# MPEGGroup/mpeg-pcc-tmc13

Hardware: AMD Instinct MI355X
Metric: RAHT forward+inverse attribute-transform Mpoints/s (bit-exact vs CPU reference) (higher is better)
Workload: dtype int64 (Q15 fixed point), int32 I/O; 1 GPU; subnode=1 pred=1 ext=1 qp34: RAHT forward+inverse, 1x1000000 Morton-sorted S-lidar/GPU, C=1; frames_per_gpu=1, roundtrip_decoder_equals_encoder_recon=True

## Files before the change

mpeg-pcc-tmc13_amd/csrc/gpcc_attr_mi355.hip:

```cpp
#include <hip/hip_runtime.h>

#include <algorithm>
#include <cstdio>
#include <cstdlib>
#include <dlfcn.h>
#include <cstring>
#include <atomic>
#include <map>
#include <mutex>
#include <thread>
#include <string>
#include <cmath>
#include <vector>

#include "gpcc_attr_mi355.h"
#include "raht_common.hpp"
#include "raht_edges.hpp"
#include "raht_levels.hpp"
#include "raht_rdoq.hpp"
#include "raht_subnode.hpp"
#include "raht_pipe.hpp"
#include "raht_sweep.hpp"
#include "raht_tile.hpp"
#include "raht_tree.hpp"
// ... 442 lines not shown
  bool links = false;
};

void
carve(Arena& ar, Plan& pl)
{
  ar.reset();
  const int n = pl.n, s = pl.s, c = pl.c, nlev = pl.nlev;
  pl.pt_off = ar.take<int32_t>(s + 1);
  pl.cap.assign(nlev, 0);
  for (int li = 0; li < nlev; li++) {
    int64_t cap = n;
    const int up = nlev - 1 - li;
    if (up < 11) {
      int64_t full = (int64_t)s << (3 * up);
      cap = std::min<int64_t>(cap, full);
    }
    pl.cap[li] = cap;
    pl.tv.cap[li] = (int32_t)cap;
    pl.tv.key[li] = ar.take<int64_t>(cap + 1);
    pl.tv.fp[li] = ar.take<int32_t>(cap + 2);
    pl.tv.fc[li] = ar.take<int32_t>(cap + 2);
    pl.tv.soff[li] = ar.take<int32_t>(s + 1);
  }
  pl.tv.nlev = nlev;
  pl.tv.num_slices = s;
  pl.tv.n_total = n;
  pl.tv.num_tiles = (n + kTilePoints - 1) / kTilePoints;
  pl.tv.pt_off = pl.pt_off;
  pl.tile_cnt = ar.take<uint32_t>((size_t)pl.tv.num_tiles * nlev);
  pl.tile_attr = ar.take<int32_t>((size_t)pl.tv.num_tiles * c);
  pl.sched = ar.take<SliceSched>(s);
  pl.worklist = ar.take<int32_t>((size_t)n + 1);
  pl.work_count = ar.take<int32_t>(kMaxLevels * 9);
  pl.scan_state = ar.take<unsigned long long>(1024);
  pl.pocc = pl.sub ? ar.take<uint8_t>((size_t)n + 1) : nullptr;
  pl.mbox = pl.sub ? ar.take<uint32_t>((size_t)n * c * 4) : nullptr;
  pl.rdoq_state = (pl.sub && pl.lossy) ? ar.take<unsigned long long>((size_t)n + 1) : nullptr;
  pl.params = ar.take<gpcc_raht_params>(1);
  for (int i = 0; i < 2; i++) {
    pl.rec[i] = ar.take<int64_t>((size_t)n * c);
    pl.rec_us[i] = ar.take<int64_t>((size_t)n * c);
    pl.nneigh[i] = ar.take<int32_t>(n);
    pl.dqp[i] = pl.has_qp ? ar.take<int32_t>((size_t)n * 2) : nullptr;
  }
  pl.attr_prefix = nullptr;
  pl.dup_hf = nullptr;
  pl.haar_lf.assign(nlev, nullptr);
  pl.asc_qp.assign(nlev, nullptr);
  pl.haar_lf_tab = nullptr;
  pl.asc_qp_tab = nullptr;
  if (pl.encoder && !pl.haar)
    pl.attr_prefix = ar.take<int32_t>(((size_t)n + 1) * c);
  if (pl.encoder && pl.haar) {
    pl.dup_hf = ar.take<int32_t>((size_t)n * c);
    pl.haar_lf_tab = ar.take<int32_t*>(nlev);
    for (int li = 0; li < nlev; li++)
      pl.haar_lf[li] = ar.take<int32_t>((size_t)(pl.cap[li] + 1) * c);
  }
  if (pl.has_qp) {
    pl.asc_qp_tab = ar.take<int32_t*>(nlev);
    for (int li = 0; li < nlev; li++)
      pl.asc_qp[li] = ar.take<int32_t>((size_t)(pl.cap[li] + 1) * 2);
  }
  pl.desc = nullptr;
  pl.ptrans = nullptr;
  if (pl.lossy) {
    pl.desc = ar.take<uint32_t>(n);
    pl.ptrans = pl.sub ? nullptr : ar.take<int64_t>((size_t)n * c);
// ... 365 lines not shown
      for (int li = 1; li < nlev; li++) {
        ac.li = li;
        ascend_level_kernel<C><<<grid_for(pl.cap[li], 256), 256, 0, st>>>(ac);
      }
      if (pl.has_qp)
        qp_root_kernel<<<(s + 63) / 64, 64, 0, st>>>(ac, pl.sched);
    }
  }

  LevelCtx lc{};
  lc.tv = tv;
  lc.params = pl.params;
  lc.sched = pl.sched;
  lc.attr_prefix = pl.attr_prefix;
  lc.haar_lf = (encoder && pl.haar) ? pl.haar_lf_tab : nullptr;
  lc.asc_qp = pl.has_qp ? pl.asc_qp_tab : nullptr;
  for (int i = 0; i < 2; i++) {
    lc.rec[i] = pl.rec[i];
    lc.rec_us[i] = pl.rec_us[i];
    lc.nneigh[i] = pl.nneigh[i];
    lc.dqp[i] = pl.dqp[i];
  }
  lc.coeffs = d_coeffs;
  lc.desc = pl.desc;
  lc.ptrans = pl.ptrans;
  lc.lut = ctx->d_lut;
  lc.worklist = pl.worklist;
  lc.work_count = pl.work_count;
  lc.scan_state = pl.scan_state;
  lc.pocc = pl.pocc;
  lc.mbox = pl.mbox;
  lc.ticket = pl.work_count + kMaxLevels;
  lc.error = ctx->d_error;
  HIP_TRY(hipMemsetAsync(pl.work_count, 0, kMaxLevels * 9 * sizeof(int32_t), st));
  HIP_TRY(hipMemsetAsync(pl.scan_state, 0, 1024 * sizeof(unsigned long long), st));
  if (pl.mbox)
    HIP_TRY(hipMemsetAsync(pl.mbox, 0, (size_t)n * C * 4 * sizeof(uint32_t), st));
  if (pl.rdoq_state)
    HIP_TRY(hipMemsetAsync(pl.rdoq_state, 0, ((size_t)n + 1) * sizeof(unsigned long long), st));
  lc.rdoq_state = pl.rdoq_state;
  lc.slice_l = pl.slice_l;

  RdoqCtx rc{};
  if (pl.lossy) {
    rc.tv = tv;
    rc.sched = pl.sched;
    rc.tile_base = pl.rtile_base;
    rc.num_tiles = pl.num_rtiles;
    rc.desc = pl.desc;
    rc.coeffs = d_coeffs;
    rc.slice_l = pl.slice_l;
    rc.state = pl.rtile_state;
    rc.c = C;
    HIP_TRY(hipMemsetAsync(pl.rtile_state, 0, ((size_t)pl.num_rtiles + 1) * sizeof(unsigned long long), st));
    HIP_TRY(hipMemsetAsync(pl.slice_l, 0xff, 2 * (size_t)s * sizeof(int32_t), st));
  }

  if (tiles) {
    lc.li = 0;
    const int cgrid = std::min(s, 2048);
    if (!encoder) {
      Timer t(ctx, "coarse_synth");
      raht_coarse_kernel<C, kCoarseDecode><<<cgrid, 1024, 0, st>>>(lc);
    } else if (pl.haar) {
      Timer t(ctx, "coarse_fused");
      raht_coarse_kernel<C, kCoarseHaar><<<cgrid, 1024, 0, st>>>(lc);
    } else {
      Timer t(ctx, "coarse_lossy");
      raht_coarse_kernel<C, kCoarseLossy><<<cgrid, 1024, 0, st>>>(lc);
    }
  }

  HIP_TRY(hipEventSynchronize(ctx->ev_stats));
  const TreeStats ts = *ctx->h_stats;
  const int first_level = std::min(nlev - 1, tiles ? ts.fine_levels : ts.max_top);

  bool piped = false;
  if (pl.pipe && first_level >= 1) {
    PipeCtx px{};
    int64_t total = 0;
    for (int li = 0; li <= first_level; li++) {
      px.uoff[li] = (int32_t)total;
      total += ts.nodes[li];
    }
    const size_t need = (size_t)total * (4 + 1 + 4 + 32 * C) + 2048;
    void* pipe_mem = nullptr;
    if (total * C * 16 < ((int64_t)1 << 31) && pool_malloc(ctx, &pipe_mem, need) == hipSuccess) {
      Arena pa;
// ... 14 lines not shown
        Timer t(ctx, "pipe_prepass");
        pipe_iota_kernel<<<grid_for(total, 256), 256, 0, st>>>(px.src, (int)total);
        for (int li = first_level - 1; li >= 0; li--) {
          lc.li = li;
          const int64_t parents = ts.nodes[li + 1];
          raht_pipe_prepass_kernel<C><<<(int)std::min<int64_t>((parents + 1023) / 1024, 1024), 256, 0, st>>>(lc, px);
        }
      }
      {
        Timer t(ctx, "pipe_synth");
        if (pl.f64)
          raht_pipe_synth_kernel<C, ArithF64><<<kSubGrid, 256, 0, st>>>(lc, px);
        else
          raht_pipe_synth_kernel<C><<<kSubGrid, 256, 0, st>>>(lc, px);
      }
      {
        Timer t(ctx, "pipe_leaf");
        pipe_leaf_kernel<C><<<grid_for(ts.nodes[0], 256), 256, 0, st>>>(lc, px);
      }
      piped = true;
      pool_free(ctx, pipe_mem);
    }
  }

  LinkSchedule links;
  auto link_prof = [&](const char* name, int li) { return Timer(ctx, li < 0 ? name : level_name(name, li)); };
  const bool use_links = pl.links && !piped && !tiles && first_level >= 1 && hp->raht_extension != 0;
  if (use_links) {
    links.tv = tv;
    links.lv = pl.lv;
    links.begin(st, ts.nodes, first_level, link_prof);
  }
  int level_from = first_level;
  static const int rec_mode = [] {
    const char* e = getenv("GPCC_REC");
    return e ? atoi(e) : 0;
  }();
  const bool ext_flag = hp->raht_extension != 0;
  const bool use_rec = pl.sub && !pl.haar && !pl.has_qp && !pl.links && !piped && rec_mode == 1;
  size_t rec_need = 0;
  if (use_rec)
    for (int li = std::min(first_level, sweep ? std::max(0, ts.fine_levels) : first_level) - 1; li >= 0; li--)
      rec_need = std::max(rec_need, sweep_rec_bytes(level_max_blocks(ts.nodes, li, ext_flag), C));
  if (sweep && !piped && ts.fine_levels < first_level) {
    const int lo = std::max(0, ts.fine_levels);
    const SweepCtx sw{first_level - 1, lo};
    SweepRec rec{};
    const int64_t sweep_parents = sweep_rec_layout(&rec, ts.nodes, sw.li_hi, sw.li_lo);
    if (ensure_sweep_mem(ctx, std::max(rec_need, sweep_rec_bytes(sweep_parents, C))) == GPCC_OK) {
      level_from = lo;
      sweep_rec_carve(&rec, ctx->sweep_mem, sweep_parents, C);
      Timer t(ctx, encoder ? "sub_sweep_lossy" : "sub_sweep_synth");
      sweep_launch<C>(st, lc, sw, rec, ts.nodes, s, encoder, pl.f64);
    }
  }
  for (int li = piped ? -1 : level_from - 1; li >= 0; li--) {
    lc.li = li;
    lc.mtag = (uint32_t)(li + 1);
    const int64_t parents = ts.nodes[li + 1];
    if (use_links) {
      links.produce(st, li + 1, link_prof);
      lc.link_rec = pl.lv.rec[(li + 1) & 1];
      lc.link_lrec = pl.lv.lrec[(li + 1) & 1];
    }
    if (tiles) {
      const bool sparse = ts.nodes[li] * 8 <= parents * 9 && parents >= 64 * kTileTSparse;
      const int tile_t = sparse ? kTileTSparse : kTileT;
      const int ntiles = (int)((parents + tile_t - 1) / tile_t);
      const int tgrid = std::min((ntiles + 7) / 8 * 8, kLevelGridMax);
#define GPCC_TILE_LAUNCH(MODE)                                                  \
  do {                                                                          \
    if (sparse)                                                                 \
      raht_tile_kernel<C, MODE, kTileTSparse><<<tgrid, kTileThreads, 0, st>>>(lc); \
    else                                                                        \
      raht_tile_kernel<C, MODE, kTileT><<<tgrid, kTileThreads, 0, st>>>(lc);    \
  } while (0)
      if (!encoder) {
        Timer t(ctx, level_name("tile_synth", li));
        GPCC_TILE_LAUNCH(kSynth);
      } else if (pl.haar) {
        Timer t(ctx, level_name("tile_fused", li));
        GPCC_TILE_LAUNCH(kFused);
      } else {
        {
          Timer t(ctx, level_name("tile_analyze", li));
          GPCC_TILE_LAUNCH(kAnalyze);
        }
        rc.li = li;
        {
          Timer t(ctx, "rdoq_resolve");
          rdoq_resolve_launch(rc, st);
        }
        {
          Timer t(ctx, level_name("tile_synth_rec", li));
          GPCC_TILE_LAUNCH(kSynthRec);
        }
      }
#undef GPCC_TILE_LAUNCH
      continue;
    }
    {
      Timer t(ctx, level_name("level_prepass", li));
      raht_level_prepass_kernel<C><<<(int)std::min<int64_t>((parents + 1023) / 1024, 1024), 256, 0, st>>>(lc);
    }
    const int sgrid = (int)std::min<int64_t>(
      kSubGrid, std::max<int64_t>(8, (parents / (GPCC_SUB_BLOCKS_PER_WG) + 7) / 8 * 8));
    lc.claim_rounds = sub_claim_rounds(encoder, pl.haar, parents);
    bool rec_level = false;
    if (use_rec && ensure_sweep_mem(ctx, rec_need) == GPCC_OK) {
      Timer t(ctx, level_name("level_record", li));
      lc.brec = level_record_launch<C>(st, lc, li, ctx->sweep_mem, level_max_blocks(ts.nodes, li, ext_flag), encoder, pl.f64);
      rec_level = true;
    }
    if (rec_level && !encoder) {
      Timer t(ctx, level_name("level_sub_synth", li));
      if (pl.f64)
        raht_level_sub_kernel<C, kSynth, ArithF64, false, true><<<sgrid, 256, 0, st>>>(lc);
      else
        raht_level_sub_kernel<C, kSynth, ArithI64, false, true><<<sgrid, 256, 0, st>>>(lc);
    } else if (rec_level) {
      Timer t(ctx, level_name("level_sub_lossy", li));
      if (pl.f64)
        raht_level_sub_kernel<C, kLossySub, ArithF64, false, true><<<sgrid, 256, 0, st>>>(lc);
      else
        raht_level_sub_kernel<C, kLossySub, ArithI64, false, true><<<sgrid, 256, 0, st>>>(lc);
    } else if (!encoder) {
      Timer t(ctx, level_name("level_sub_synth", li));
      if (pl.f64)
        raht_level_sub_kernel<C, kSynth, ArithF64><<<sgrid, 256, 0, st>>>(lc);
      else
        raht_level_sub_kernel<C, kSynth><<<sgrid, 256, 0, st>>>(lc);
    } else if (pl.haar) {
      Timer t(ctx, level_name("level_sub_fused", li));
      raht_level_sub_kernel<C, kFused><<<sgrid, 256, 0, st>>>(lc);
// ... 3206 lines not shown
    while ((int64_t(3) << (shift << 1)) < dist2 && shift < 20)
      ++shift;
    *shift_bits = shift;
  } while (0);
  pool_free(ctx, d_xyz);
  pool_free(ctx, d_dist);
  return rc;
}

}

#if GPCC_FIN_VAR == 2
extern "C" int
gpcc_debug_fin(unsigned int* out, int reset)
{
  if (hipMemcpyFromSymbol(out, HIP_SYMBOL(gpcc::g_fin_dbg), sizeof(gpcc::g_fin_dbg)) != hipSuccess)
    return -1;
  if (reset) {
    unsigned int z[4 + 4 * 60] = {};
    if (hipMemcpyToSymbol(HIP_SYMBOL(gpcc::g_fin_dbg), z, sizeof(z)) != hipSuccess)
      return -1;
  }
  return 0;
}
#endif

#ifdef GPCC_SUB_PROF
extern "C" int
gpcc_debug_sub_prof(unsigned long long* out, int reset)
{
  if (hipMemcpyFromSymbol(out, HIP_SYMBOL(gpcc::g_sub_prof), sizeof(gpcc::g_sub_prof)) != hipSuccess)
    return -1;
  if (reset) {
    static unsigned long long z[16 + 32 * 20] = {};
    if (hipMemcpyToSymbol(HIP_SYMBOL(gpcc::g_sub_prof), z, sizeof(z)) != hipSuccess)
      return -1;
  }
  return 0;
}
#endif

#ifdef GPCC_PIPE_PROF
extern "C" int
gpcc_debug_pipe_prof(unsigned long long* out, int reset)
{
  if (hipMemcpyFromSymbol(out, HIP_SYMBOL(gpcc::g_pipe_prof), sizeof(gpcc::g_pipe_prof)) != hipSuccess)
    return -1;
  if (reset) {
    static unsigned long long z[32 * 8] = {};
    if (hipMemcpyToSymbol(HIP_SYMBOL(gpcc::g_pipe_prof), z, sizeof(z)) != hipSuccess)
      return -1;
  }
  return 0;
}
#endif

#ifdef GPCC_TILE_PROF
extern "C" int
gpcc_debug_tile_prof(unsigned long long* out, int reset)
{
  if (hipMemcpyFromSymbol(out, HIP_SYMBOL(gpcc::g_tile_prof), sizeof(gpcc::g_tile_prof)) != hipSuccess)
    return -1;
  if (reset) {
    static unsigned long long z[5 * 24 * 8] = {};
    if (hipMemcpyToSymbol(HIP_SYMBOL(gpcc::g_tile_prof), z, sizeof(z)) != hipSuccess)
      return -1;
  }
// ... 2676 lines not shown
```

mpeg-pcc-tmc13_amd/csrc/raht_levels.hpp:

```cpp
#pragma once

#include "raht_common.hpp"

namespace gpcc {

enum LevelMode { kAnalyze = 0, kSynth = 1, kFused = 2, kLossySub = 3 };

constexpr uint32_t kDescNever = 0x7fffffffu;
constexpr uint32_t kDescZero = 0x80000000u;

typedef const __attribute__((address_space(4))) gpcc_raht_params* ParamsConst;

struct InterRef {
  const int64_t* pos;
  const int32_t* prefix;
  int32_t n_ref;
  int32_t lr;
  int32_t blocks;
  int32_t dual;
  int32_t filtered;
  const int32_t* tap;
  const int64_t* hkey;
  const int32_t* hfp;
  const int32_t* hlf;
// ... 20 lines not shown


struct LevelCtx {
  TreeView tv;
  const gpcc_raht_params* params;
  const SliceSched* sched;
  const int32_t* attr_prefix;
  const int32_t* const* haar_lf;
  const int32_t* const* asc_qp;
  int64_t* rec[2];
  int64_t* rec_us[2];
  int32_t* nneigh[2];
  int32_t* dqp[2];
  int32_t* coeffs;
  uint32_t* desc;
  int64_t* ptrans;
  int32_t li;
  const struct SharedLut* lut;
  int32_t* worklist;
  int32_t* work_count;
  unsigned long long* scan_state;
  uint8_t* pocc;
  uint32_t* mbox;
  uint32_t mtag;
  int32_t* ticket;
  int32_t* error;
  unsigned long long* rdoq_state;
  int32_t* slice_l;
  InterRef inter;
  const int32_t* link_rec;
  const int32_t* link_lrec;
  int32_t claim_rounds;
  SweepRec brec;
};

template<typename T>
__device__ __forceinline__ T*
par2(T* const (&a)[2], int p)
{
  const ptrdiff_t d = a[1] - a[0];
  return a[0] + (p ? d : (ptrdiff_t)0);
}

constexpr int kSmallW = 16;
constexpr int kSmallN = 64;

struct SharedLut {
  RsqrtLut rsqrt;
  int32_t bfly_a[kSmallW * kSmallW];
  int32_t bfly_b[kSmallW * kSmallW];
  int32_t norm_rs[kSmallN];
  int32_t norm_sq[kSmallN];
};

__device__ __forceinline__ void
raht_coeffs_slow(int32_t wl, int32_t wr, const RsqrtLut& lut, int64_t* a, int64_t* b)
{
  const uint64_t rs = irsqrt((uint64_t)wl + (uint64_t)wr, lut);
  *a = (int64_t)(((uint64_t)isqrt((uint64_t)wl << 30, lut) * rs) >> 40);
  *b = (int64_t)(((uint64_t)isqrt((uint64_t)wr << 30, lut) * rs) >> 40);
}

__global__ __launch_bounds__(256) void
lut_init_kernel(SharedLut* g)
{
  __shared__ RsqrtLut rs;
// ... 265 lines not shown
          const int pt0 = tv.pt_off[s];
          const int64_t prow = (int64_t)pt0 + (j - tv.soff[li + 1][s]);
          const int64_t crow = (int64_t)pt0 + (c0 - tv.soff[li][s]);
          const int pp = e.parity ^ 1, cp = e.parity;
#pragma unroll
          for (int k = 0; k < C; k++) {
            par2(ctx.rec_us, cp)[crow * C + k] = par2(ctx.rec_us, pp)[prow * C + k];
            par2(ctx.rec, cp)[crow * C + k] = par2(ctx.rec, pp)[prow * C + k];
          }
          par2(ctx.nneigh, cp)[crow] = 19;
          if (ctx.asc_qp) {
            par2(ctx.dqp, cp)[crow * 2] = par2(ctx.dqp, pp)[prow * 2];
            par2(ctx.dqp, cp)[crow * 2 + 1] = par2(ctx.dqp, pp)[prow * 2 + 1];
          }
        } else {
          real = true;
        }
      }
    }
    const unsigned long long m = __ballot(real);
    __syncthreads();
    if (lane == 0)
      wave_cnt[wave] = __popcll(m);
    __syncthreads();
    int off = running;
    for (int w = 0; w < wave; w++)
      off += wave_cnt[w];
    if (real)
      ctx.worklist[off + __popcll(m & ((1ull << lane) - 1))] = j;
    running += wave_cnt[0] + wave_cnt[1] + wave_cnt[2] + wave_cnt[3];
  }
}

}
```

mpeg-pcc-tmc13_amd/csrc/raht_subnode.hpp:

```cpp
#pragma once

#include <stdlib.h>

#include "raht_arith.hpp"
#include "raht_inter.hpp"
#include "raht_levels.hpp"
#include "raht_links.hpp"

namespace gpcc {

#ifndef GPCC_SUB_CHUNK
#define GPCC_SUB_CHUNK 1
#endif
#ifndef GPCC_SUB_DSTORE
#define GPCC_SUB_DSTORE 0
#endif
__device__ __forceinline__ int64_t
sub_round_of_ticket(int tk, int cls)
{
  constexpr int K = GPCC_SUB_CHUNK;
  return ((int64_t)(tk / K) * 8 + cls) * K + tk % K;
}

#ifdef GPCC_SUB_PROF
__device__ unsigned long long g_sub_prof[16 + 32 * 20];
struct SubProf {
  unsigned long long t0 = 0, t1 = 0, last = 0, acc[4] = {0, 0, 0, 0}, iters = 0, idle_iters = 0;
  unsigned long long last2 = 0, sub_acc[6] = {0, 0, 0, 0, 0, 0}, execs[2] = {0, 0};
  template<int WHICH> __device__ void enter() { execs[WHICH]++; last2 = now(); }
  template<int K> __device__ void sub() { const unsigned long long t = now(); sub_acc[K] += t - last2; last2 = t; }
  __device__ static unsigned long long now() { return __builtin_amdgcn_s_memtime(); }
  __device__ void round_begin() { t0 = now(); }
  __device__ void loop_begin() { t1 = now(); }
  __device__ void iter_begin() { last = now(); iters++; }
  template<int STAGE> __device__ void mark() { const unsigned long long t = now(); acc[STAGE] += t - last; last = t; }
  __device__ void idle() { idle_iters++; }
  __device__ void round_end(int lane, int li)
  {
    if (lane != 0)
      return;
    const unsigned long long t2 = now();
    const unsigned long long v[9] = {1, t1 - t0, t2 - t1, acc[0], acc[1], acc[2], acc[3], iters, idle_iters};
    for (int i = 0; i < 9; i++)
      atomicAdd(&g_sub_prof[i], v[i]);
    atomicAdd(&g_sub_prof[16 + li * 4 + 0], 1ull);
    atomicAdd(&g_sub_prof[16 + li * 4 + 1], t1 - t0);
    atomicAdd(&g_sub_prof[16 + li * 4 + 2], t2 - t1);
    atomicAdd(&g_sub_prof[16 + li * 4 + 3], iters);
    for (int i = 0; i < 4; i++)
      atomicAdd(&g_sub_prof[144 + li * 6 + i], acc[i]);
    atomicAdd(&g_sub_prof[144 + li * 6 + 4], idle_iters);
    atomicAdd(&g_sub_prof[336 + li * 10 + 0], execs[0]);
    atomicAdd(&g_sub_prof[336 + li * 10 + 1], execs[1]);
    for (int i = 0; i < 6; i++)
      atomicAdd(&g_sub_prof[336 + li * 10 + 2 + i], sub_acc[i]);
  }
};
#else
struct SubProf {
  __device__ void round_begin() {}
  __device__ void loop_begin() {}
  __device__ void iter_begin() {}
  template<int STAGE> __device__ void mark() {}
  template<int WHICH> __device__ void enter() {}
  template<int K> __device__ void sub() {}
  __device__ void idle() {}
  __device__ void round_end(int, int) {}
};
#endif

inline int
sub_claim_rounds(bool encoder, bool haar, int64_t parents)
{
#if GPCC_EXPERIMENTS
  auto rounds = [] {
    const char* e = getenv("GPCC_SUB_CLAIM");
    const int v = e ? atoi(e) : 1;
    return v < 1 ? 1 : (v > 64 ? 64 : v);
  };
  auto limit = [] {
    const char* e = getenv("GPCC_SUB_CLAIM_PARENTS");
    return e ? (int64_t)atoll(e) : (int64_t)100000;
  };
#ifdef GPCC_EMU
  const int r = rounds();
  const int64_t lim = limit();
#else
  static const int r = rounds();
  static const int64_t lim = limit();
#endif
  return (encoder && !haar && r > 1 && parents <= lim) ? r : 1;
#else
  (void)encoder;
  (void)haar;
  (void)parents;
  return 1;
#endif
}

__device__ __forceinline__ int
occu_shift(int i12)
{
  constexpr uint8_t s[12] = {6, 5, 4, 3, 2, 1, 3, 1, 2, 1, 2, 3};
  return s[i12];
}

__device__ __forceinline__ int32_t
load_agent_i32(const int32_t* p)
{
  return __hip_atomic_load(p, __ATOMIC_RELAXED, __HIP_MEMORY_SCOPE_AGENT);
}
__device__ __forceinline__ int64_t
load_agent_i64(const int64_t* p)
{
  return __hip_atomic_load(p, __ATOMIC_RELAXED, __HIP_MEMORY_SCOPE_AGENT);
}
__device__ __forceinline__ void
store_agent_i64(int64_t* p, int64_t v)
{
  __hip_atomic_store(p, v, __ATOMIC_RELAXED, __HIP_MEMORY_SCOPE_AGENT);
}

#ifndef GPCC_SUB_SLEEP
#define GPCC_SUB_SLEEP 4
#endif
#ifndef GPCC_SUB_LOSSY_WAVES
#define GPCC_SUB_LOSSY_WAVES 3
#endif
#ifndef GPCC_SUB_SYNTH3_WAVES
#define GPCC_SUB_SYNTH3_WAVES 4
#endif
// ... 18 lines not shown
  const TreeView& tv = ctx.tv;
  const ParamsConst prm = (ParamsConst)ctx.params;
  const int li = ctx.li;
  const int t = threadIdx.x & 7;
  const int lane = lane_id();
  const int gbase = threadIdx.x & 56;
  const bool haar = !A::kF64 && prm->integer_haar_enable_flag != 0;
  const bool ext = A::kF64 || prm->raht_extension != 0;
  const int32_t epoch = li + 1;
#ifdef GPCC_EMU
  __shared__ unsigned long long wmail_s[8 * 4 * 64 * C];
  unsigned long long* wm = wmail_s + ((blockIdx.x & 7) * 4 + (threadIdx.x >> 6)) * (64 * C);
#else
  __shared__ unsigned long long wmail_s[4 * 64 * C];
  unsigned long long* wm = wmail_s + (threadIdx.x >> 6) * (64 * C);
#endif
#ifdef GPCC_EMU
  __shared__ int32_t nrow_s[8][12][256];
  __shared__ int32_t pwc_s[8 * 4][12];
#define GPCC_SUB_NROW(i12) nrow_s[blockIdx.x & 7][i12][threadIdx.x]
#define GPCC_SUB_PWC(i12) pwc_s[(blockIdx.x & 7) * 4 + (threadIdx.x >> 6)][i12]
#else
  __shared__ int32_t nrow_s[12][256];
  __shared__ int32_t pwc_s[4][12];
#define GPCC_SUB_NROW(i12) nrow_s[i12][threadIdx.x]
#define GPCC_SUB_PWC(i12) pwc_s[threadIdx.x >> 6][i12]
#endif
  if (lane < 12)
    GPCC_SUB_PWC(lane) = prm->pred_weight_child[lane];
  bool in_range = true;
  const int cls = blockIdx.x & 7;

  const int num_work = ctx.work_count[li];
#if GPCC_EXPERIMENTS
  const int claim_rounds = ctx.claim_rounds > 1 ? ctx.claim_rounds : 1;
  bool stop_all = false;
  for (;;) {
    int tk = 0;
    if (lane == 0)
      tk = atomicAdd(&ctx.ticket[li * 8 + (claim_rounds > 1 ? 0 : cls)], 1);
    tk = __shfl(tk, 0);
    const int64_t wround0 = claim_rounds > 1 ? (int64_t)tk * claim_rounds : sub_round_of_ticket(tk, cls);
    if (wround0 * 8 >= num_work || stop_all)
      break;
    bool carry_known = false;
    int carry_l = -1;
   for (int sr = 0; sr < claim_rounds; sr++) {
    const int64_t wround = wround0 + sr;
    if (wround * 8 >= num_work)
      break;
    SubProf prof;
    prof.round_begin();
    if (__hip_atomic_load(ctx.error, __ATOMIC_RELAXED, __HIP_MEMORY_SCOPE_AGENT)) {
      stop_all = true;
      break;
    }
#else
  for (;;) {
    int tk = 0;
    if (lane == 0)
      tk = atomicAdd(&ctx.ticket[li * 8 + cls], 1);
    tk = __shfl(tk, 0);
    const int64_t wround = sub_round_of_ticket(tk, cls);
    if (wround * 8 >= num_work)
      break;
    SubProf prof;
// ... 434 lines not shown
      }
    }

    int nb_c0[3] = {0, 0, 0};
    uint32_t nb_occ[3] = {0, 0, 0};
    int nb_single[3] = {0, 0, 0};
    VT nb_v[3][C];
#pragma unroll
    for (int slot = 0; slot < 3; slot++) {
#pragma unroll
      for (int k = 0; k < C; k++)
        nb_v[slot][k] = A::zero();
      const int i = 1 + t + 8 * slot;
      if (run && i >= 7 && i < 19 && pn[slot] >= 0) {
        const int q = pn[slot];
#pragma unroll
        for (int k = 0; k < C; k++) {
          nb_v[slot][k] = A::from_i64(prec[(rbase + q) * C + k]);
          in_range = in_range && A::below(nb_v[slot][k], A::kRecLimit);
        }
        if constexpr (REC) {
          nb_c0[slot] = rf[(kSfNbc0 + slot) * rln];
          nb_occ[slot] = (rpk >> (8 * slot)) & 0xffu;
          nb_single[slot] = (int)((rpk >> (24 + slot)) & 1u);
        } else if (q < j) {
          const int qc0 = tv.fc[li + 1][q];
          nb_c0[slot] = qc0;
          nb_occ[slot] = ctx.pocc[q];
          nb_single[slot] = ext && tv.fc[li + 1][q + 1] - qc0 == 1;
        }
      }
    }
    uint32_t pend = 0;
    uint32_t inw = 0, wsrc_a = 0, wsrc_b = 0;
    int jg[8];
#pragma unroll
    for (int g = 0; g < 8; g++)
      jg[g] = __shfl(on ? j : -1, g << 3);
#pragma unroll
    for (int i12 = 0; i12 < 12; i12++) {
      const int i = 7 + i12;
      const int owner = gbase | ((i - 1) & 7);
      const int sl = (i - 1) >> 3;
      const int q = __shfl(pn[sl], owner);
      const int qc0 = __shfl(nb_c0[sl], owner);
      const uint32_t qocc = __shfl(nb_occ[sl], owner);
      const int single = __shfl(nb_single[sl], owner);
      VT v[C];
#pragma unroll
      for (int k = 0; k < C; k++)
        v[k] = shfl_v(nb_v[sl][k], owner);
      if (!run || q < 0)
        continue;
      if (A::muli(v[0], 10) <= lim_lo || A::muli(v[0], 10) >= lim_hi)
        continue;
      if (has && ((neigh_mask(i) >> t) & 1)) {
        const int sh = occu_shift(i12);
        const int cpos = i12 < 9 ? t + sh : t - sh;
        const bool child_ok = cpos >= 0 && cpos < 8 && ((qocc >> cpos) & 1);
        if (child_ok) {
          const int cidx_n = qc0 + popc32(qocc & ((1u << cpos) - 1));
          const int64_t nrow = (int64_t)pt0 + (cidx_n - sc0);
          const int pwc = prm->pred_weight_child[i12];
          wsum += pwc;
          if (single) {
            const int mul = ext ? pwc : (pwc << kFpFrac);
#pragma unroll
            for (int k = 0; k < C; k++) {
              const VT cv = A::from_i64(par2(ctx.rec, cur_par)[nrow * C + k]);
              in_range = in_range && A::below(cv, A::kRecLimit);
              pred[k] += A::muli(cv, mul);
            }
          } else {
            GPCC_SUB_NROW(i12) = (int32_t)nrow;
            pend |= 1u << i12;
            int pg = -1;
#pragma unroll
            for (int g = 0; g < 7; g++)
              pg = q == jg[g] ? g : pg;
            if (pg >= 0) {
              inw |= 1u << i12;
              if (i12 < 10)
                wsrc_a |= (uint32_t)pg << (3 * i12);
              else
                wsrc_b |= (uint32_t)pg << (3 * (i12 - 10));
            }
          }
        } else {
          const int pwp = prm->pred_weight_parent[i];
          wsum += pwp;
          const int mul = ext ? pwp : (pwp << kFpFrac);
#pragma unroll
          for (int k = 0; k < C; k++)
            pred[k] += A::muli(v[k], mul);
        }
      }
    }
    const VC pdiv = A::coef(pred_divisor(wsum > 0 ? wsum : 1));
    const auto mrsrc = __builtin_amdgcn_make_buffer_rsrc(
      ctx.mbox, 0, (int)((size_t)tv.n_total * C * 16), 0x00020000);

    bool use_inter = false;
    VT ipin[C];
#pragma unroll
    for (int k = 0; k < C; k++)
      ipin[k] = A::zero();
    if constexpr (INTER) {
      if (ctx.inter.blocks) {
        bool node;
        int64_t pin[C];
        if (ctx.inter.hkey)
          inter_block_haar<C>(ctx.inter, on ? tv.key[li + 1][j] : 0, t, on, &node, pin);
        else
          inter_block<C>(ctx.inter, on ? tv.key[li + 1][j] : 0, t, on, lut, &node, pin);
        use_inter = node;
#pragma unroll
        for (int k = 0; k < C; k++) {
          ipin[k] = A::from_i64(pin[k]);
          in_range = in_range && (!node || A::below(ipin[k], A::kFwdLimit));
        }
        if (use_inter) {
          pend = 0;
          inw = 0;
          enable_pred = on;
        }
      }
    }

    int stage = on ? 0 : 3;
    unsigned spins = 0;
    VT pt[C];
    int32_t qc[C];
    uint32_t dr = kDescZero;
    int zs = 0;
    bool zero_r = false;
    uint32_t dmask = 0;
    bool lin_exact = false;
    int need = 0;
    int look = wi - 1;
    int outk = 0, outv = -1;
    unsigned long long done = 0;
    unsigned long long done_seen = ~0ull;
    int cur_slot = -1, cur_pwc = 0;
    int32_t cur_row = 0;
#pragma unroll
    for (int k = 0; k < C; k++) {
      pt[k] = A::zero();
      qc[k] = (!kEnc && coded) ? cplane[(size_t)k * n_s] : 0;
    }
#ifndef GPCC_EMU
    __builtin_amdgcn_s_waitcnt(0x0f70);
#endif
    prof.loop_begin();
    while (__any(stage != 3)) {
      bool progressed = false;
      prof.iter_begin();
      if (done != done_seen) {
        done_seen = done;
        uint32_t mi = stage == 0 ? (pend & inw) : 0u;
        while (__any(mi != 0)) {
          const bool act = mi != 0;
          const int slot = act ? __ffs(mi) - 1 : 0;
          mi &= mi - 1;
          const uint32_t pg = (slot < 10 ? wsrc_a >> (3 * slot) : wsrc_b >> (3 * (slot - 10))) & 7u;
          constexpr unsigned long long kShifts = 06ull | 05ull << 3 | 04ull << 6 | 03ull << 9 | 02ull << 12
            | 01ull << 15 | 03ull << 18 | 01ull << 21 | 02ull << 24 | 01ull << 27 | 02ull << 30 | 03ull << 33;
          const int sh = (int)((kShifts >> (3 * slot)) & 7);
          const int srcl = (int)(pg << 3) | ((slot < 9 ? t + sh : t - sh) & 7);
          if (act && ((done >> srcl) & 1)) {
            const int pwc = GPCC_SUB_PWC(slot);
            const int mul = ext ? pwc : (pwc << kFpFrac);
#pragma unroll
            for (int k = 0; k < C; k++)
              pred[k] += A::muli(__builtin_bit_cast(VT, wm[srcl * C + k]), mul);
            pend &= ~(1u << slot);
            inw &= ~(1u << slot);
          }
        }
      }
      const uint32_t pm = stage == 0 ? (pend & ~inw) : 0u;
      u32x4 g[C];
      if (pm) {
        const int slot = __ffs(pm) - 1;
        if (slot != cur_slot) {
          cur_slot = slot;
          cur_row = GPCC_SUB_NROW(slot);
          cur_pwc = GPCC_SUB_PWC(slot);
        }
#pragma unroll
        for (int k = 0; k < C; k++)
          g[k] = __builtin_amdgcn_raw_buffer_load_b128(mrsrc, (cur_row * C + k) * 16, 0,  16);
      }
      auto take_poll = [&]() -> bool {
        bool ok = pm != 0;
        if (pm) {
#pragma unroll
          for (int k = 0; k < C; k++) {
#ifndef GPCC_EMU
            asm volatile("" : : "v"(g[k]));
#endif
            ok = ok && g[k].z == ctx.mtag;
          }
          if (ok) {
            const int mul = ext ? cur_pwc : (cur_pwc << kFpFrac);
#pragma unroll
            for (int k = 0; k < C; k++)
              pred[k] += A::muli(__builtin_bit_cast(VT, ((uint64_t)g[k].y << 32) | g[k].x), mul);
            pend &= ~(1u << cur_slot);
          }
        }
        return ok;
      };
      bool blocked = group8_any(stage == 0 && pend);
      bool poll_open = __any(stage == 0 && !blocked);
      if (!poll_open) {
        if (__any(take_poll()))
          blocked = group8_any(stage == 0 && pend);
      }
      auto take_poll_behind = [&]() {
#ifndef GPCC_EMU
        __builtin_amdgcn_s_waitcnt(0x0f70);
#endif
        if (poll_open)
          take_poll();
      };
      prof.mark<0>();
      const bool nready = stage == 0 && !blocked;

      if (__any(nready)) {
        progressed = true;
        prof.template enter<0>();
        VT pw_[C];
#pragma unroll
        for (int k = 0; k < C; k++)
          pw_[k] = pred[k];
        if (run && has) {
#pragma unroll
          for (int k = 0; k < C; k++) {
            pw_[k] = A::mulc(pw_[k], pdiv);
            if constexpr (!A::kF64) {
              if (haar)
                pw_[k] = (pw_[k] >> kFpFrac) << kFpFrac;
            }
          }
        }
        if (!haar && w > 1 && enable_pred) {
#pragma unroll
          for (int k = 0; k < C; k++)
            pw_[k] = A::mulc(pw_[k], nrm_sq);
        }
#pragma unroll
        for (int k = 0; k < C; k++)
          in_range = in_range && A::below(pw_[k], A::kFwdLimit);
#pragma unroll
        for (int st = 0; st < 3; st++) {
          const int bit = 1 << st;
          const bool left = !(t & bit);
          const bool both = wl[st] && wr[st];
          const bool swap = !wl[st] && wr[st];
#pragma unroll
          for (int k = 0; k < C; k++) {
            const VT own = pw_[k], oth = shfl_xor_v(own, bit);
            if constexpr (A::kF64) {
              const VT bf = A::mulc(own, ca[st]) + A::mulc(left ? oth : -oth, cb[st]);
// ... 313 lines not shown
      if (!kLossy)
        take_poll_behind();
      if (__any(can)) {
        if (can && has) {
          VT vn[C];
#pragma unroll
          for (int k = 0; k < C; k++) {
            VT v = pw_[k];
            if (!haar && w > 1)
              v = A::mulc(A::shr(v, nrm_shift), nrm_rs);
            v = ext ? v : A::round_int(v);
            vn[k] = v;
            const uint64_t vb = __builtin_bit_cast(uint64_t, v);
            wm[lane * C + k] = vb;
            const u32x4 gr = {(uint32_t)vb, (uint32_t)(vb >> 32), ctx.mtag, 0u};
#if GPCC_SUB_DSTORE
            __builtin_amdgcn_raw_buffer_store_b128(gr, mrsrc, (int)((crow * C + k) * 16), 0, 0);
#endif
            __builtin_amdgcn_raw_buffer_store_b128(gr, mrsrc, (int)((crow * C + k) * 16), 0,  16);
          }
          prof.template sub<3>();
#pragma unroll
          for (int k = 0; k < C; k++) {
            par2(ctx.rec_us, cur_par)[crow * C + k] = A::to_i64(ext ? pw_[k] : A::round_int(A::muli(pw_[k], 4)));
            par2(ctx.rec, cur_par)[crow * C + k] = A::to_i64(vn[k]);
          }
          par2(ctx.nneigh, cur_par)[crow] = inherit_dc ? neigh_count : 19;
          prof.template sub<4>();
        }
        if (can)
          stage = 3;
      }

      done |= __ballot(can && has);
      prof.mark<3>();
      if (!progressed) {
        prof.idle();
        if (++spins > (1u << 21)) {
          if (lane == 0)
            atomicExch(ctx.error, 1);
          break;
        }
        __builtin_amdgcn_s_sleep(GPCC_SUB_SLEEP);
      }
    }
    prof.round_end(lane, li);
#if GPCC_EXPERIMENTS
    if (kLossy && claim_rounds > 1) {
      const unsigned long long fin = __ballot(outk == 2) & 0x0101010101010101ull;
      if (fin) {
        carry_l = __shfl(outv, 63 - __clzll((long long)fin));
        carry_known = true;
      } else if (__any(outk == 1)) {
        carry_known = false;
      }
    }
   }
#endif
  }
  if (A::kF64 && __any(!in_range) && lane == 0)
    atomicCAS(ctx.error, 0, 3);
#undef GPCC_SUB_NROW
#undef GPCC_SUB_PWC
}

}
```

Baseline: 101.3 Mpoints/s.

## Plan all RAHT levels in one kernel and copy single-child nodes in tail

Adds a single up-front planning kernel that builds per-level worklists and child-occupancy bytes for every level, using a decoupled look-back scan. This replaces the per-level prepass launches. Single-child parents are left out of the worklist, and the subnode kernel copies them with a ticketed, ILP-unrolled tail copy, also propagating slice_l for lossy mode. The single-neighbour prediction now reuses already-shuffled neighbour values instead of reloading rec, which drops the in-range check on that path. The planning kernel needs larger scan and pocc buffers and relies on cross-block spinning.

After: 97.28 Mpoints/s. 0.96x the previous value.

```diff
diff --git a/mpeg-pcc-tmc13_amd/csrc/gpcc_attr_mi355.hip b/mpeg-pcc-tmc13_amd/csrc/gpcc_attr_mi355.hip
--- a/mpeg-pcc-tmc13_amd/csrc/gpcc_attr_mi355.hip
+++ b/mpeg-pcc-tmc13_amd/csrc/gpcc_attr_mi355.hip
@@ -498,9 +498,9 @@
   pl.tile_attr = ar.take<int32_t>((size_t)pl.tv.num_tiles * c);
   pl.sched = ar.take<SliceSched>(s);
   pl.worklist = ar.take<int32_t>((size_t)n + 1);
-  pl.work_count = ar.take<int32_t>(kMaxLevels * 9);
-  pl.scan_state = ar.take<unsigned long long>(1024);
-  pl.pocc = pl.sub ? ar.take<uint8_t>((size_t)n + 1) : nullptr;
+  pl.work_count = ar.take<int32_t>(kMaxLevels * 17);
+  pl.scan_state = ar.take<unsigned long long>((size_t)kMaxLevels * kPlanScanRow);
+  pl.pocc = pl.sub ? ar.take<uint8_t>(std::max<size_t>((size_t)n + 1, (size_t)plan_pocc_offset(pl.tv.cap, nlev - 1) + 1)) : nullptr;
   pl.mbox = pl.sub ? ar.take<uint32_t>((size_t)n * c * 4) : nullptr;
   pl.rdoq_state = (pl.sub && pl.lossy) ? ar.take<unsigned long long>((size_t)n + 1) : nullptr;
   pl.params = ar.take<gpcc_raht_params>(1);
@@ -932,8 +932,16 @@
   lc.mbox = pl.mbox;
   lc.ticket = pl.work_count + kMaxLevels;
   lc.error = ctx->d_error;
-  HIP_TRY(hipMemsetAsync(pl.work_count, 0, kMaxLevels * 9 * sizeof(int32_t), st));
-  HIP_TRY(hipMemsetAsync(pl.scan_state, 0, 1024 * sizeof(unsigned long long), st));
+  static const int rec_mode = [] {
+    const char* e = getenv("GPCC_REC");
+    return e ? atoi(e) : 0;
+  }();
+  const bool ext_flag = hp->raht_extension != 0;
+  const bool planned = pl.sub && ext_flag && !pl.pipe && !pl.links && rec_mode != 1
+    && sub_claim_rounds(encoder, pl.haar, 0) == 1;
+  HIP_TRY(hipMemsetAsync(pl.work_count, 0, kMaxLevels * 17 * sizeof(int32_t), st));
+  HIP_TRY(hipMemsetAsync(
+    pl.scan_state, 0, (planned ? (size_t)nlev * kPlanScanRow : (size_t)kPlanScanRow) * sizeof(unsigned long long), st));
   if (pl.mbox)
     HIP_TRY(hipMemsetAsync(pl.mbox, 0, (size_t)n * C * 4 * sizeof(uint32_t), st));
   if (pl.rdoq_state)
@@ -954,6 +962,11 @@
     rc.c = C;
     HIP_TRY(hipMemsetAsync(pl.rtile_state, 0, ((size_t)pl.num_rtiles + 1) * sizeof(unsigned long long), st));
     HIP_TRY(hipMemsetAsync(pl.slice_l, 0xff, 2 * (size_t)s * sizeof(int32_t), st));
+  }
+
+  if (planned) {
+    Timer t(ctx, "level_plan");
+    raht_plan_levels_kernel<C><<<(int)std::min<int64_t>(((int64_t)n + 1023) / 1024, 1024), 256, 0, st>>>(lc);
   }
 
   if (tiles) {
@@ -1034,11 +1047,6 @@
     links.begin(st, ts.nodes, first_level, link_prof);
   }
   int level_from = first_level;
-  static const int rec_mode = [] {
-    const char* e = getenv("GPCC_REC");
-    return e ? atoi(e) : 0;
-  }();
-  const bool ext_flag = hp->raht_extension != 0;
   const bool use_rec = pl.sub && !pl.haar && !pl.has_qp && !pl.links && !piped && rec_mode == 1;
   size_t rec_need = 0;
   if (use_rec)
@@ -1101,7 +1109,11 @@
 #undef GPCC_TILE_LAUNCH
       continue;
     }
-    {
+    if (planned) {
+      lc.worklist = pl.worklist + plan_worklist_offset(ts.nodes[li + 1], ts.nodes[nlev - 1]);
+      lc.pocc = pl.pocc + plan_pocc_offset(pl.tv.cap, li);
+      lc.tail = 1;
+    } else {
       Timer t(ctx, level_name("level_prepass", li));
       raht_level_prepass_kernel<C><<<(int)std::min<int64_t>((parents + 1023) / 1024, 1024), 256, 0, st>>>(lc);
     }
diff --git a/mpeg-pcc-tmc13_amd/csrc/raht_levels.hpp b/mpeg-pcc-tmc13_amd/csrc/raht_levels.hpp
--- a/mpeg-pcc-tmc13_amd/csrc/raht_levels.hpp
+++ b/mpeg-pcc-tmc13_amd/csrc/raht_levels.hpp
@@ -76,6 +76,7 @@
   const int32_t* link_lrec;
   int32_t claim_rounds;
   SweepRec brec;
+  int32_t tail;
 };
 
 template<typename T>
@@ -407,4 +408,228 @@
   }
 }
 
-}
+__host__ __device__ inline int64_t
+plan_worklist_offset(int64_t nodes_parents, int64_t nodes_top)
+{
+  return nodes_parents - nodes_top;
+}
+__host__ __device__ inline int64_t
+plan_pocc_offset(const int32_t* cap, int li)
+{
+  int64_t o = 0;
+  for (int l = 0; l < li; l++)
+    o += (int64_t)cap[l + 1] + 1;
+  return o;
+}
+constexpr int kPlanScanRow = 1024;
+
+constexpr int kTailIlp = 4;
+constexpr int kTailChunk = kTailIlp * kWave;
+
+template<int C>
+__device__ __forceinline__ void
+level_copy_single_children(const LevelCtx& ctx, int li, int64_t j0, int lane, int num_parents)
+{
+  const TreeView& tv = ctx.tv;
+  bool one[kTailIlp];
+  int64_t prow[kTailIlp], crow[kTailIlp];
+  int cp[kTailIlp];
+#pragma unroll
+  for (int u = 0; u < kTailIlp; u++) {
+    const int64_t jj = j0 + lane + u * kWave;
+    const bool ok = jj < num_parents;
+    const int j = ok ? (int)jj : 0;
+    const int s = find_slice(tv.soff[li + 1], tv.num_slices, j);
+    const LevelSched e = ctx.sched[s].lvl[li];
+    const int c0 = tv.fc[li + 1][j];
+    const int c1 = tv.fc[li + 1][j + 1];
+    const int pt0 = tv.pt_off[s];
+    one[u] = ok && e.processed && c1 - c0 == 1;
+    prow[u] = (int64_t)pt0 + (j - tv.soff[li + 1][s]);
+    crow[u] = (int64_t)pt0 + (c0 - tv.soff[li][s]);
+    cp[u] = e.parity;
+  }
+  int64_t us[kTailIlp][C], sc[kTailIlp][C];
+  int32_t q0[kTailIlp], q1[kTailIlp];
+#pragma unroll
+  for (int u = 0; u < kTailIlp; u++) {
+    q0[u] = q1[u] = 0;
+#pragma unroll
+    for (int k = 0; k < C; k++)
+      us[u][k] = sc[u][k] = 0;
+    if (one[u]) {
+#pragma unroll
+      for (int k = 0; k < C; k++) {
+        us[u][k] = par2(ctx.rec_us, cp[u] ^ 1)[prow[u] * C + k];
+        sc[u][k] = par2(ctx.rec, cp[u] ^ 1)[prow[u] * C + k];
+      }
+      if (ctx.asc_qp) {
+        q0[u] = par2(ctx.dqp, cp[u] ^ 1)[prow[u] * 2];
+        q1[u] = par2(ctx.dqp, cp[u] ^ 1)[prow[u] * 2 + 1];
+      }
+    }
+  }
+#pragma unroll
+  for (int u = 0; u < kTailIlp; u++) {
+    if (one[u]) {
+#pragma unroll
+      for (int k = 0; k < C; k++) {
+        par2(ctx.rec_us, cp[u])[crow[u] * C + k] = us[u][k];
+        par2(ctx.rec, cp[u])[crow[u] * C + k] = sc[u][k];
+      }
+      par2(ctx.nneigh, cp[u])[crow[u]] = 19;
+      if (ctx.asc_qp) {
+        par2(ctx.dqp, cp[u])[crow[u] * 2] = q0[u];
+        par2(ctx.dqp, cp[u])[crow[u] * 2 + 1] = q1[u];
+      }
+    }
+  }
+}
+
+constexpr int kPlanIlp = 4;
+
+template<int C>
+__global__ __launch_bounds__(256) void
+raht_plan_levels_kernel(LevelCtx ctx)
+{
+  GPCC_VGPR_FLOOR_64();
+  __shared__ int wave_cnt[kPlanIlp][4];
+  __shared__ int base_s;
+  if (tree_failed(ctx.tv))
+    return;
+  const TreeView& tv = ctx.tv;
+  const bool ext = ctx.params->raht_extension != 0;
+  const int lane = lane_id(), wave = threadIdx.x >> 6;
+  const int64_t nodes_top = tv.soff[tv.nlev - 1][tv.num_slices];
+  for (int li = tv.nlev - 2; li >= 0; li--) {
+    const int num_parents = tv.soff[li + 1][tv.num_slices];
+    const int64_t seg = (int64_t)tv.soff[li][tv.num_slices] - num_parents;
+    int32_t* __restrict__ worklist = ctx.worklist + plan_worklist_offset(num_parents, nodes_top);
+    uint8_t* __restrict__ pocc = ctx.pocc + plan_pocc_offset(tv.cap, li);
+    unsigned long long* scan = ctx.scan_state + (size_t)li * kPlanScanRow;
+    const int32_t* __restrict__ fc = tv.fc[li + 1];
+    const int64_t* __restrict__ key = tv.key[li];
+    const int64_t chunks = ((int64_t)num_parents + 255) >> 8;
+    const int64_t per = (chunks + gridDim.x - 1) / gridDim.x;
+    const int active = per ? (int)((chunks + per - 1) / per) : 0;
+    if ((int)blockIdx.x >= active)
+      continue;
+    const int64_t gbeg = (int64_t)blockIdx.x * per;
+    const int64_t gend = min(gbeg + per, chunks);
+
+    int mine = 0;
+    for (int64_t chunk = gbeg; chunk < gend; chunk += kPlanIlp) {
+#pragma unroll
+      for (int u = 0; u < kPlanIlp; u++) {
+        const int64_t jj = (chunk + u) * 256 + threadIdx.x;
+        const bool ok = chunk + u < gend && jj < num_parents;
+        const int j = ok ? (int)jj : 0;
+        const int s = find_slice(tv.soff[li + 1], tv.num_slices, j);
+        const bool proc = ctx.sched[s].lvl[li].processed != 0;
+        const int nchild = fc[j + 1] - fc[j];
+        mine += ok && proc && !(ext && nchild == 1);
+      }
+    }
+#pragma unroll
+    for (int d = 1; d < kWave; d <<= 1)
+      mine += __shfl_xor(mine, d);
+    __syncthreads();
+    if (lane == 0)
+      wave_cnt[0][wave] = mine;
+    __syncthreads();
+    if (wave == 0) {
+      const unsigned long long ep = (unsigned long long)(li + 1) << 48;
+      const unsigned total = wave_cnt[0][0] + wave_cnt[0][1] + wave_cnt[0][2] + wave_cnt[0][3];
+      unsigned excl = 0;
+      if (blockIdx.x > 0) {
+        if (lane == 0)
+          __hip_atomic_store(&scan[blockIdx.x], ep | (1ull << 32) | total, __ATOMIC_RELAXED, __HIP_MEMORY_SCOPE_AGENT);
+        int base = (int)blockIdx.x - 1;
+        while (base >= 0) {
+          const int k = base - lane;
+          unsigned long long v = 0;
+          if (k >= 0)
+            v = __hip_atomic_load(&scan[k], __ATOMIC_RELAXED, __HIP_MEMORY_SCOPE_AGENT);
+          const bool valid = k >= 0 && (v >> 48) == (unsigned long long)(li + 1);
+          const unsigned long long inv = __ballot(k >= 0 && !valid);
+          const unsigned long long fin = __ballot(valid && ((v >> 32) & 0xffff) == 2);
+          const int first_inv = inv ? __ffsll((long long)inv) - 1 : kWave;
+          const int first_fin = fin ? __ffsll((long long)fin) - 1 : kWave;
+          if (first_inv < first_fin) {
+            __builtin_amdgcn_s_sleep(2);
+            continue;
+          }
+          unsigned part = (valid && lane <= first_fin) ? (unsigned)v : 0u;
+#pragma unroll
+          for (int d = 1; d < kWave; d <<= 1)
+            part += __shfl_xor(part, d);
+          excl += part;
+          if (first_fin < kWave)
+            break;
+          base -= kWave;
+        }
+      }
+      if (lane == 0) {
+        __hip_atomic_store(&scan[blockIdx.x], ep | (2ull << 32) | (excl + total), __ATOMIC_RELAXED, __HIP_MEMORY_SCOPE_AGENT);
+        if ((int)blockIdx.x == active - 1) {
+          ctx.work_count[li] = (int64_t)(excl + total) <= seg ? (int)(excl + total) : 0;
+          if ((int64_t)(excl + total) > seg)
+            atomicExch(ctx.error, 1);
+        }
+        base_s = (int)excl;
+      }
+    }
+    __syncthreads();
+    int running = base_s;
+
+    for (int64_t chunk = gbeg; chunk < gend; chunk += kPlanIlp) {
+      int j[kPlanIlp], c0[kPlanIlp], nchild[kPlanIlp];
+      bool proc[kPlanIlp];
+#pragma unroll
+      for (int u = 0; u < kPlanIlp; u++) {
+        const int64_t jj = (chunk + u) * 256 + threadIdx.x;
+        const bool ok = chunk + u < gend && jj < num_parents;
+        j[u] = ok ? (int)jj : 0;
+        const int s = find_slice(tv.soff[li + 1], tv.num_slices, j[u]);
+        proc[u] = ok && ctx.sched[s].lvl[li].processed != 0;
+        const int a = fc[j[u]], b = fc[j[u] + 1];
+        c0[u] = proc[u] ? a : 0;
+        nchild[u] = proc[u] ? b - a : 0;
+      }
+      unsigned long long m[kPlanIlp];
+      bool real[kPlanIlp];
+#pragma unroll
+      for (int u = 0; u < kPlanIlp; u++) {
+        uint32_t o = 0;
+#pragma unroll
+        for (int t = 0; t < 8; t++) {
+          const int64_t k8 = key[c0[u] + (t < nchild[u] ? t : 0)];
+          o |= t < nchild[u] ? 1u << (int)(k8 & 7) : 0u;
+        }
+        if (proc[u])
+          pocc[j[u]] = (uint8_t)o;
+        real[u] = proc[u] && !(ext && nchild[u] == 1);
+        m[u] = __ballot(real[u]);
+      }
+      __syncthreads();
+      if (lane == 0) {
+#pragma unroll
+        for (int u = 0; u < kPlanIlp; u++)
+          wave_cnt[u][wave] = __popcll(m[u]);
+      }
+      __syncthreads();
+#pragma unroll
+      for (int u = 0; u < kPlanIlp; u++) {
+        int off = running;
+        for (int w = 0; w < wave; w++)
+          off += wave_cnt[u][w];
+        const int at = off + __popcll(m[u] & ((1ull << lane) - 1));
+        if (real[u] && at < seg)
+          worklist[at] = j[u];
+        running += wave_cnt[u][0] + wave_cnt[u][1] + wave_cnt[u][2] + wave_cnt[u][3];
+      }
+    }
+  }
+}
+
+}
diff --git a/mpeg-pcc-tmc13_amd/csrc/raht_subnode.hpp b/mpeg-pcc-tmc13_amd/csrc/raht_subnode.hpp
--- a/mpeg-pcc-tmc13_amd/csrc/raht_subnode.hpp
+++ b/mpeg-pcc-tmc13_amd/csrc/raht_subnode.hpp
@@ -181,6 +181,24 @@
   const int cls = blockIdx.x & 7;
 
   const int num_work = ctx.work_count[li];
+  if (kLossy && ctx.tail && ctx.slice_l && blockIdx.x == 0)
+    for (int s = threadIdx.x; s < tv.num_slices; s += blockDim.x)
+      atomicMax(&ctx.slice_l[(li & 1) * tv.num_slices + s], ctx.slice_l[((li + 1) & 1) * tv.num_slices + s]);
+  auto copy_tail = [&]() {
+    const int num_parents = tv.soff[li + 1][tv.num_slices];
+    for (;;) {
+      int tk = 0;
+      if (lane == 0)
+        tk = atomicAdd(&ctx.ticket[kMaxLevels * 8 + li * 8 + cls], 1);
+      tk = __shfl(tk, 0);
+      const int64_t j0 = ((int64_t)tk * 8 + cls) * kTailChunk;
+      if (j0 >= num_parents)
+        break;
+      level_copy_single_children<C>(ctx, li, j0, lane, num_parents);
+    }
+  };
+  if (ctx.tail && ext && ((blockIdx.x >> 3) & 3) == 3)
+    copy_tail();
 #if GPCC_EXPERIMENTS
   const int claim_rounds = ctx.claim_rounds > 1 ? ctx.claim_rounds : 1;
   bool stop_all = false;
@@ -715,11 +733,8 @@
           if (single) {
             const int mul = ext ? pwc : (pwc << kFpFrac);
 #pragma unroll
-            for (int k = 0; k < C; k++) {
-              const VT cv = A::from_i64(par2(ctx.rec, cur_par)[nrow * C + k]);
-              in_range = in_range && A::below(cv, A::kRecLimit);
-              pred[k] += A::muli(cv, mul);
-            }
+            for (int k = 0; k < C; k++)
+              pred[k] += A::muli(v[k], mul);
           } else {
             GPCC_SUB_NROW(i12) = (int32_t)nrow;
             pend |= 1u << i12;
@@ -1284,6 +1299,8 @@
    }
 #endif
   }
+  if (ctx.tail && ext)
+    copy_tail();
   if (A::kF64 && __any(!in_range) && lane == 0)
     atomicCAS(ctx.error, 0, 3);
 #undef GPCC_SUB_NROW
```

## Drive mailbox consumption from newly committed groups instead of rescanning pending slots

Applied to the files above, without the earlier changes.

Replaces the done-bitmask rescan, which walked every pending in-wave slot whenever any lane committed, with a queue of newly committed 8-lane groups. A 4-bit-per-group table maps each group to the slot waiting on it, so each iteration only visits groups that just finished. The goal is less per-iteration wavefront work in the subnode spin loop. It also adds profiling counters and emulator statistics, and it assumes at most one waiting slot per source group.

New measurement: 101.3 Mpoints/s before, 106.2 Mpoints/s after (median of 6 runs). 4.8% higher.

```diff
diff --git a/mpeg-pcc-tmc13_amd/csrc/gpcc_attr_mi355.hip b/mpeg-pcc-tmc13_amd/csrc/gpcc_attr_mi355.hip
--- a/mpeg-pcc-tmc13_amd/csrc/gpcc_attr_mi355.hip
+++ b/mpeg-pcc-tmc13_amd/csrc/gpcc_attr_mi355.hip
@@ -4374,7 +4374,7 @@
   if (hipMemcpyFromSymbol(out, HIP_SYMBOL(gpcc::g_sub_prof), sizeof(gpcc::g_sub_prof)) != hipSuccess)
     return -1;
   if (reset) {
-    static unsigned long long z[16 + 32 * 20] = {};
+    static unsigned long long z[sizeof(gpcc::g_sub_prof) / sizeof(unsigned long long)] = {};
     if (hipMemcpyToSymbol(HIP_SYMBOL(gpcc::g_sub_prof), z, sizeof(z)) != hipSuccess)
       return -1;
   }
diff --git a/mpeg-pcc-tmc13_amd/csrc/raht_subnode.hpp b/mpeg-pcc-tmc13_amd/csrc/raht_subnode.hpp
--- a/mpeg-pcc-tmc13_amd/csrc/raht_subnode.hpp
+++ b/mpeg-pcc-tmc13_amd/csrc/raht_subnode.hpp
@@ -23,10 +23,22 @@
 }
 
 #ifdef GPCC_SUB_PROF
-__device__ unsigned long long g_sub_prof[16 + 32 * 20];
+__device__ unsigned long long g_sub_prof[16 + 32 * 28];
 struct SubProf {
   unsigned long long t0 = 0, t1 = 0, last = 0, acc[4] = {0, 0, 0, 0}, iters = 0, idle_iters = 0;
   unsigned long long last2 = 0, sub_acc[6] = {0, 0, 0, 0, 0, 0}, execs[2] = {0, 0};
+  unsigned long long walk_acc = 0, walk_execs = 0, walk_trips = 0, fed[3] = {0, 0, 0};
+  __device__ void walk_end(bool ran, int trips)
+  {
+    if (!ran)
+      return;
+    const unsigned long long t = now();
+    walk_acc += t - last;
+    last = t;
+    walk_execs += ran;
+    walk_trips += trips;
+  }
+  __device__ void fed_by(bool any_poll, bool any_mailbox) { fed[any_poll ? 2 : (any_mailbox ? 1 : 0)]++; }
   template<int WHICH> __device__ void enter() { execs[WHICH]++; last2 = now(); }
   template<int K> __device__ void sub() { const unsigned long long t = now(); sub_acc[K] += t - last2; last2 = t; }
   __device__ static unsigned long long now() { return __builtin_amdgcn_s_memtime(); }
@@ -54,6 +66,11 @@
     atomicAdd(&g_sub_prof[336 + li * 10 + 1], execs[1]);
     for (int i = 0; i < 6; i++)
       atomicAdd(&g_sub_prof[336 + li * 10 + 2 + i], sub_acc[i]);
+    atomicAdd(&g_sub_prof[656 + li * 8 + 0], walk_execs);
+    atomicAdd(&g_sub_prof[656 + li * 8 + 1], walk_trips);
+    atomicAdd(&g_sub_prof[656 + li * 8 + 2], walk_acc);
+    for (int i = 0; i < 3; i++)
+      atomicAdd(&g_sub_prof[656 + li * 8 + 3 + i], fed[i]);
   }
 };
 #else
@@ -65,6 +82,7 @@
   template<int WHICH> __device__ void enter() {}
   template<int K> __device__ void sub() {}
   __device__ void idle() {}
+  __device__ void walk_end(bool, int) {}
   __device__ void round_end(int, int) {}
 };
 #endif
@@ -97,6 +115,13 @@
   return 1;
 #endif
 }
+
+#ifdef GPCC_EMU
+extern "C" {
+inline int gpcc_emu_sub_max_commits = 0;
+inline int gpcc_emu_sub_max_taken = 0;
+}
+#endif
 
 __device__ __forceinline__ int
 occu_shift(int i12)
@@ -681,7 +706,7 @@
       }
     }
     uint32_t pend = 0;
-    uint32_t inw = 0, wsrc_a = 0, wsrc_b = 0;
+    uint32_t inw = 0, wtab = 0;
     int jg[8];
 #pragma unroll
     for (int g = 0; g < 8; g++)
@@ -729,10 +754,7 @@
               pg = q == jg[g] ? g : pg;
             if (pg >= 0) {
               inw |= 1u << i12;
-              if (i12 < 10)
-                wsrc_a |= (uint32_t)pg << (3 * i12);
-              else
-                wsrc_b |= (uint32_t)pg << (3 * (i12 - 10));
+              wtab |= (uint32_t)(i12 + 1) << (4 * pg);
             }
           }
         } else {
@@ -788,10 +810,12 @@
     int need = 0;
     int look = wi - 1;
     int outk = 0, outv = -1;
-    unsigned long long done = 0;
-    unsigned long long done_seen = ~0ull;
+    unsigned long long newg = 0;
     int cur_slot = -1, cur_pwc = 0;
     int32_t cur_row = 0;
+#ifdef GPCC_SUB_PROF
+    bool got_mb = false, got_poll = false;
+#endif
 #pragma unroll
     for (int k = 0; k < C; k++) {
       pt[k] = A::zero();
@@ -804,29 +828,41 @@
     while (__any(stage != 3)) {
       bool progressed = false;
       prof.iter_begin();
-      if (done != done_seen) {
-        done_seen = done;
-        uint32_t mi = stage == 0 ? (pend & inw) : 0u;
-        while (__any(mi != 0)) {
-          const bool act = mi != 0;
-          const int slot = act ? __ffs(mi) - 1 : 0;
-          mi &= mi - 1;
-          const uint32_t pg = (slot < 10 ? wsrc_a >> (3 * slot) : wsrc_b >> (3 * (slot - 10))) & 7u;
-          constexpr unsigned long long kShifts = 06ull | 05ull << 3 | 04ull << 6 | 03ull << 9 | 02ull << 12
-            | 01ull << 15 | 03ull << 18 | 01ull << 21 | 02ull << 24 | 01ull << 27 | 02ull << 30 | 03ull << 33;
-          const int sh = (int)((kShifts >> (3 * slot)) & 7);
-          const int srcl = (int)(pg << 3) | ((slot < 9 ? t + sh : t - sh) & 7);
-          if (act && ((done >> srcl) & 1)) {
-            const int pwc = GPCC_SUB_PWC(slot);
-            const int mul = ext ? pwc : (pwc << kFpFrac);
-#pragma unroll
-            for (int k = 0; k < C; k++)
-              pred[k] += A::muli(__builtin_bit_cast(VT, wm[srcl * C + k]), mul);
-            pend &= ~(1u << slot);
-            inw &= ~(1u << slot);
-          }
-        }
-      }
+      int prof_trips = 0;
+      const bool prof_ran = newg != 0;
+#ifdef GPCC_EMU
+      int emu_taken = 0;
+#endif
+      while (newg) {
+        const int gl = __ffsll((long long)newg) - 1;
+        newg &= newg - 1;
+        prof_trips++;
+        const uint32_t s1 = (wtab >> (gl >> 1)) & 15u;
+        const uint32_t bit = (1u << s1) >> 1;
+        if (pend & bit) {
+          constexpr unsigned long long kDelta = 06ull << 3 | 05ull << 6 | 04ull << 9 | 03ull << 12 | 02ull << 15 | 01ull << 18
+            | 03ull << 21 | 01ull << 24 | 02ull << 27 | 07ull << 30 | 06ull << 33 | 05ull << 36;
+          const int srcl = gl | ((t + (int)(kDelta >> (3 * s1))) & 7);
+          const int pwc = GPCC_SUB_PWC((int)s1 - 1);
+          const int mul = ext ? pwc : (pwc << kFpFrac);
+#pragma unroll
+          for (int k = 0; k < C; k++)
+            pred[k] += A::muli(__builtin_bit_cast(VT, wm[srcl * C + k]), mul);
+          pend &= ~bit;
+          inw &= ~bit;
+#ifdef GPCC_SUB_PROF
+          got_mb = true;
+#endif
+#ifdef GPCC_EMU
+          emu_taken++;
+#endif
+        }
+      }
+#ifdef GPCC_EMU
+      if (emu_taken > gpcc_emu_sub_max_taken)
+        gpcc_emu_sub_max_taken = emu_taken;
+#endif
+      prof.walk_end(prof_ran, prof_trips);
       const uint32_t pm = stage == 0 ? (pend & ~inw) : 0u;
       u32x4 g[C];
       if (pm) {
@@ -856,6 +892,9 @@
             for (int k = 0; k < C; k++)
               pred[k] += A::muli(__builtin_bit_cast(VT, ((uint64_t)g[k].y << 32) | g[k].x), mul);
             pend &= ~(1u << cur_slot);
+#ifdef GPCC_SUB_PROF
+            got_poll = true;
+#endif
           }
         }
         return ok;
@@ -879,6 +918,12 @@
       if (__any(nready)) {
         progressed = true;
         prof.template enter<0>();
+#ifdef GPCC_SUB_PROF
+        {
+          const bool gp = group8_any(got_poll), gm = group8_any(got_mb);
+          prof.fed_by(__any(nready && gp), __any(nready && gm));
+        }
+#endif
         VT pw_[C];
 #pragma unroll
         for (int k = 0; k < C; k++)
@@ -1258,7 +1303,11 @@
           stage = 3;
       }
 
-      done |= __ballot(can && has);
+      newg |= __ballot(can && t == 0);
+#ifdef GPCC_EMU
+      if (__popcll(newg) > gpcc_emu_sub_max_commits)
+        gpcc_emu_sub_max_commits = __popcll(newg);
+#endif
       prof.mark<3>();
       if (!progressed) {
         prof.idle();
```
